# daooshee/ReReVST-Code

Hardware: AMD Instinct MI355X
Metric: stylized frames/sec at 512x512, 1 style (higher is better)
Workload: dtype f32

## Files before the change

### rerevst-code_amd/csrc/rerevst_hip.hip

```cpp
#include <hip/hip_runtime.h>
#include <dlfcn.h>
#include <stddef.h>
#include <stdint.h>
#include <string.h>
#include <algorithm>
#include <cmath>
#include <thread>
#include <stdio.h>
#include <map>
#include <condition_variable>
#include <mutex>
#include <string>
#include <vector>

#include "../../include/rerevst_hip.h"
#include "conv_mfma.h"
#include "conv_wino.h"
#include "conv_wino_split.h"
#include "conv_f43.h"
#include "conv_thin.h"
#include "prep_kernels.h"
#include "mask_kernels.h"

namespace {
// ... 174 lines not shown
    struct Ticket { long id = -1; void* out = nullptr; size_t out_bytes = 0; bool open = false; } tickets[4];
    long next_ticket = 0;
    int grid_share = 1;
    int f43_mode = 1;
    unsigned f43_layers = F43_DEFAULT_LAYERS;
    bool illcond = false;
    bool enc_p8_tables = false;
    int p8 = 3;
    bool f43_path = false;
    unsigned direct_layers = 0;
    int ms_group = 0;
    int host_io = 0;
    int n_cus = 256;
    int debug = 0;
    int fail_alloc_in = 0;
    bool profiling = false;
    std::vector<ProfEntry> prof;
};

namespace {

#define HIPCHK(expr)                                                                              \
    do {                                                                                          \
        hipError_t _e = (expr);                                                                   \
        if (_e != hipSuccess) {                                                                   \
            char _b[512];                                                                         \
            snprintf(_b, sizeof _b, "%s failed: %s (%s:%d)", #expr, hipGetErrorString(_e), __FILE__, __LINE__); \
            h->err = _b;                                                                          \
            return _e == hipErrorOutOfMemory ? RRV_E_NOMEM : RRV_E_HIP;                           \
        }                                                                                         \
    } while (0)
#define RCHK(expr) do { int _r = (expr); if (_r != RRV_OK) return _r; } while (0)

int fail(rrv_handle h, int code, const std::string& msg) { h->err = msg; return code; }
int dmalloc(rrv_handle h, void** p, size_t bytes);

int check_image_size(rrv_handle h, double H, double W, const char* who) {
    if ((H + 2) * (W + 2) * 64.0 < 2147483648.0) return RRV_OK;
    return fail(h, RRV_E_ARG, std::string(who) + ": frame too large ((H+2)*(W+2)*64 must be < 2^31)");
}
int check_frame(rrv_handle h, int H, int W, const char* who) {
    if (H < 8 || W < 8) return fail(h, RRV_E_ARG, std::string(who) + ": frames must be at least 8 x 8 pixels");
    return check_image_size(h, H, W, who);
}

int sync_all(rrv_handle h) {
    for (int i = 0; i < RRV_MAX_SLOTS; ++i)
        if (h->streams[i]) HIPCHK(hipStreamSynchronize(h->streams[i]));
    if (h->copy_in) HIPCHK(hipStreamSynchronize(h->copy_in));
    if (h->copy_out) HIPCHK(hipStreamSynchronize(h->copy_out));
    return RRV_OK;
}

int dmalloc(rrv_handle h, void** p, size_t bytes) {
    *p = nullptr;
    if (h->fail_alloc_in > 0 && --h->fail_alloc_in == 0) {
        char b[160];
        snprintf(b, sizeof b, "out of device memory (injected by rrv_debug_fail_alloc) allocating %zu bytes", bytes);
        return fail(h, RRV_E_NOMEM, b);
    }
    const hipError_t e = hipMalloc(p, bytes);
    if (e != hipSuccess) {
        (void)hipGetLastError();
        *p = nullptr;
        char b[200];
        snprintf(b, sizeof b, "hipMalloc of %zu bytes failed: %s", bytes, hipGetErrorString(e));
        return fail(h, e == hipErrorOutOfMemory ? RRV_E_NOMEM : RRV_E_HIP, b);
    }
    return RRV_OK;
}

int dalloc(rrv_handle h, float** p, size_t floats, bool zero = true) {
    RCHK(dmalloc(h, (void**)p, floats * sizeof(float)));
    if (zero) HIPCHK(hipMemsetAsync(*p, 0, floats * sizeof(float), h->stream));
    return RRV_OK;
}

constexpr size_t DBG_GUARD = 16384;
constexpr uint32_t DBG_CANARY = 0xDEADBEEFu;
struct DbgRec { rrv_ctx* h; float* base; int B, H, W, C; size_t floats; };
std::mutex g_dbg_mu;
std::map<float*, DbgRec> g_dbg;

__global__ void dbg_check_k(const float* base, const float* p, int B, int H, int W, int C, size_t floats, unsigned* counters) {
    const uint32_t* gb = (const uint32_t*)base;
    const uint32_t* u = (const uint32_t*)p;
    const size_t img = (size_t)(H + 2) * (W + 2) * C;
    const size_t tid = blockIdx.x * (size_t)blockDim.x + threadIdx.x, nth = (size_t)gridDim.x * blockDim.x;
    unsigned bad_guard = 0, bad_ring = 0;
    for (size_t i = tid; i < DBG_GUARD; i += nth) bad_guard += (gb[i] != DBG_CANARY) + (((const uint32_t*)(p + floats))[i] != DBG_CANARY);
    const size_t ring_px = (size_t)2 * (W + 2) + (size_t)2 * H;
    for (size_t i = tid; i < (size_t)B * ring_px * C; i += nth) {
        const size_t c = i % C, r = (i / C) % ring_px, b = i / C / ring_px;
        size_t y, x;
        if (r < (size_t)(W + 2)) { y = 0; x = r; }
        else if (r < (size_t)2 * (W + 2)) { y = H + 1; x = r - (W + 2); }
        else { const size_t q = r - 2 * (W + 2); y = 1 + (q >> 1); x = (q & 1) ? W + 1 : 0; }
        bad_ring += u[b * img + (y * (W + 2) + x) * C + c] != 0u;
    }
    for (size_t i = (size_t)B * img + tid; i < floats; i += nth) bad_ring += u[i] != 0u;
    if (bad_guard) atomicAdd(&counters[0], bad_guard);
    if (bad_ring) atomicAdd(&counters[1], bad_ring);
}
__global__ void dbg_fill_k(uint32_t* p, size_t n, uint32_t v) {
    for (size_t i = blockIdx.x * (size_t)blockDim.x + threadIdx.x; i < n; i += (size_t)gridDim.x * blockDim.x) p[i] = v;
}
// ... 1217 lines not shown
    if (rc == RRV_OK && h->debug) rc = debug_verify(h, "Decoder.compute (streaming)");
    (void)hipStreamSynchronize(h->stream);
    h->active_src = -1;
    if (rc == RRV_OK) S.computed = true;
    if (rc == RRV_OK) rc = filter_conditioning(h, S);
    return rc;
}

}

extern "C" {

static int cu_mask_count(const char* env, int device, int n_cus) {
    if (!env || !*env) return 0;
    auto parse_list = [](const char* b, const char* e, int limit, std::vector<char>& hit) {
        hit.assign((size_t)limit, 0);
        while (b < e) {
            char* q = nullptr;
            long lo = strtol(b, &q, 10), hi = lo;
            if (q == b) return false;
            if (q < e && *q == '-') { const char* r = q + 1; hi = strtol(r, &q, 10); if (q == r) return false; }
            for (long v = lo; v <= hi; ++v) if (v >= 0 && v < limit) hit[(size_t)v] = 1;
            b = (q < e && *q == ',') ? q + 1 : q;
            if (b < e && q == b) return false;
        }
        return true;
    };
    const char* p = env;
    while (*p) {
        const char* semi = strchr(p, ';');
        const char* end = semi ? semi : p + strlen(p);
        const char* colon = (const char*)memchr(p, ':', (size_t)(end - p));
        if (colon) {
            std::vector<char> gpus, cus;
            if (parse_list(p, colon, 64, gpus) && device < 64 && gpus[(size_t)device] && parse_list(colon + 1, end, n_cus, cus)) {
                int n = 0;
                for (char c : cus) n += c;
                return n;
            }
        }
        p = semi ? semi + 1 : end;
    }
    return 0;
}

int rrv_create(int device, rrv_handle* out) {
    if (!out) return RRV_E_ARG;
    *out = nullptr;
    int n = 0;
    if (hipGetDeviceCount(&n) != hipSuccess || device < 0 || device >= n) return RRV_E_HIP;
    rrv_ctx* h = new rrv_ctx();
    h->dev = device;
    bool ok = hipSetDevice(device) == hipSuccess;
    for (int i = 0; ok && i < RRV_MAX_SLOTS; ++i) ok = hipStreamCreateWithFlags(&h->streams[i], hipStreamNonBlocking) == hipSuccess;
    if (!ok) {
        delete h;
        return RRV_E_HIP;
    }
    h->stream = h->streams[0];
    ok = ok && hipStreamCreateWithFlags(&h->copy_in, hipStreamNonBlocking) == hipSuccess && hipStreamCreateWithFlags(&h->copy_out, hipStreamNonBlocking) == hipSuccess;
    for (int i = 0; ok && i < RRV_MAX_SLOTS; ++i) ok = hipEventCreateWithFlags(&h->slot_ev[i], hipEventDisableTiming) == hipSuccess;
    for (auto& st : h->hstage)
        for (hipEvent_t* e : {&st.in_done, &st.k_done, &st.out_done}) ok = ok && hipEventCreateWithFlags(e, hipEventDisableTiming) == hipSuccess;
    for (const ConvKey& e : WINO_TABLE)
        if (ok && e.attr) ok = e.attr() == hipSuccess;
    for (const ConvKey& e : F43_TABLE)
        if (ok && e.attr) ok = e.attr() == hipSuccess;
    for (const F43LayKey& e : F43_LAY_TABLE)
        if (ok && e.attr) ok = e.attr() == hipSuccess;
    if (!ok) {
        delete h;
        return RRV_E_HIP;
    }
    {
        hipDeviceProp_t prop;
        if (hipGetDeviceProperties(&prop, device) == hipSuccess && prop.multiProcessorCount > 0) h->n_cus = prop.multiProcessorCount;
        const int masked = cu_mask_count(getenv("HSA_CU_MASK"), device, h->n_cus);
        if (masked > 0 && masked < h->n_cus) h->n_cus = masked;
        if (const char* e = getenv("RRV_CUS")) { const int n = atoi(e); if (n >= 1 && n <= 1024) h->n_cus = n; }
    }
    if (const char* e = getenv("RRV_F43_LAYERS")) h->f43_layers = (unsigned)strtoul(e, nullptr, 0);
    if (const char* e = getenv("RRV_DIRECT_LAYERS")) h->direct_layers = (unsigned)strtoul(e, nullptr, 0);
    if (const char* e = getenv("RRV_P8")) h->p8 = atoi(e) & 3;
    if (const char* e = getenv("RRV_F43")) h->f43_mode = atoi(e) < 0 ? 0 : (atoi(e) > 2 ? 2 : atoi(e));
    if (const char* e = getenv("RRV_DEBUG")) h->debug = atoi(e) < 0 ? 0 : (atoi(e) > 2 ? 2 : atoi(e));
    *out = h;
    return RRV_OK;
}

static void free_plans(rrv_handle h) {
    for (auto& pair : h->enc_frame) for (EncPlan& e : pair) enc_free(e);
    enc_free(h->enc_add); enc_free(h->enc_style);
    for (auto& pair : h->dec) for (DecPlan& d : pair) dec_free(h, d);
    prep_free(h);
}

int rrv_set_debug(rrv_handle h, int level) {
    if (!h || level < 0 || level > 2) return RRV_E_ARG;
    HIPCHK(hipSetDevice(h->dev));
    RCHK(sync_all(h));
    free_plans(h);
    h->debug = level;
    return RRV_OK;
}

int rrv_debug_fail_alloc(rrv_handle h, int nth) {
    if (!h || nth < 0) return RRV_E_ARG;
    h->fail_alloc_in = nth;
    return RRV_OK;
}

__global__ void dbg_poke_k(float* p, long off) { p[off] = 1.0f; }
int rrv_debug_selftest(rrv_handle h) {
    if (!h) return RRV_E_ARG;
// ... 16 lines not shown
    h->debug = saved;
    if (rc != RRV_OK) return rc;
    if (caught != 2) return fail(h, RRV_E_DEBUG, "debug selftest: a deliberate out-of-bounds store was not detected");
    h->err.clear();
    return RRV_OK;
}

int rrv_destroy(rrv_handle h) {
    if (!h) return RRV_E_ARG;
    (void)hipSetDevice(h->dev);
    (void)hipDeviceSynchronize();
    for (auto& kv : h->conv) {
        if (kv.second.raw) (void)hipFree(kv.second.raw);
        if (kv.second.pk) (void)hipFree(kv.second.pk);
        if (kv.second.pk_ups) (void)hipFree(kv.second.pk_ups);
        if (kv.second.pk_ups_sc) (void)hipFree(kv.second.pk_ups_sc);
        if (kv.second.pk_wino) (void)hipFree(kv.second.pk_wino);
        if (kv.second.pk_f43) (void)hipFree(kv.second.pk_f43);
        if (kv.second.bias && kv.second.bias != h->zero_bias) (void)hipFree(kv.second.bias);
    }
    if (h->zero_bias) (void)hipFree(h->zero_bias);
    for (int f = 0; f < 3; ++f) {
        const ConvW &fd = h->sets[0].fold_down[f], &fu = h->sets[0].fold_up[f];
        for (float* q : {fd.raw, fd.bias, fd.pk_wino, fu.raw, fu.pk_wino}) if (q) (void)hipFree(q);
    }
    if (h->sets[0].active) (void)hipFree(h->sets[0].active);
    for (int i = 0; i < 6; ++i) { if (h->fc_w[i]) (void)hipFree(h->fc_w[i]); if (h->fc_b[i]) (void)hipFree(h->fc_b[i]); }
    if (h->fold_tmp) (void)hipFree(h->fold_tmp);
    for (float* p : h->patches) (void)hipFree(p);
    for (auto& f : h->features) if (f.owned) { if (f.p) (void)hipFree(f.p); if (f.u8) (void)hipFree(f.u8); }
    for (void* b : h->feat_blocks) (void)hipFree(b);
    free_plans(h);
    for (StyleState& s : h->styles) { if (s.blob) (void)hipFree(s.blob); if (s.smean) (void)hipFree(s.smean); tfree(&s.map); }
    if (h->d_u8) (void)hipFree(h->d_u8);
    if (h->d_outf) (void)hipFree(h->d_outf);
    if (h->pend_u8) (void)hipFree(h->pend_u8);
    for (auto& bw : h->blend_w) {
        if (bw.dev) (void)hipFree(bw.dev);
        if (bw.pin) (void)hipHostFree(bw.pin);
        for (hipEvent_t e : bw.ev) if (e) (void)hipEventDestroy(e);
    }
    if (h->stat_part) (void)hipFree(h->stat_part);
    for (float* q : {h->first_w[0], h->first_w[1], h->first_b[0], h->first_b[1], h->first_wg}) if (q) (void)hipFree(q);
    for (auto& st : h->hstage) {
        stage_free(st.pin, true);
        stage_free(st.dev, false);
        if (st.mask) (void)hipFree(st.mask);
        if (st.mask_pin) (void)hipHostFree(st.mask_pin);
        for (hipEvent_t e : {st.in_done, st.k_done, st.out_done}) if (e) (void)hipEventDestroy(e);
    }
    if (h->copy_in) (void)hipStreamDestroy(h->copy_in);
    if (h->copy_out) (void)hipStreamDestroy(h->copy_out);
    for (ProfEntry& e : h->prof) { (void)hipEventDestroy(e.e0); (void)hipEventDestroy(e.e1); }
    for (int i = 0; i < RRV_MAX_SLOTS; ++i) { (void)hipStreamDestroy(h->streams[i]); if (h->slot_ev[i]) (void)hipEventDestroy(h->slot_ev[i]); }
    delete h;
    return RRV_OK;
}

const char* rrv_last_error(rrv_handle h) { return h ? h->err.c_str() : "null handle"; }

int rrv_load_weight(rrv_handle h, const char* key, const float* data, const int64_t* shape, int ndim) {
    if (!h || !key || !data || !shape || ndim < 1 || ndim > 4) return RRV_E_ARG;
    if (h->finalized) return fail(h, RRV_E_WEIGHTS, "weights already finalized");
    size_t n = 1;
    for (int i = 0; i < ndim; ++i) n *= (size_t)shape[i];
    h->hostw[key].assign(data, data + n);
    h->hostshape[key].assign(shape, shape + ndim);
    return RRV_OK;
}

int rrv_finalize_weights(rrv_handle h) {
    if (!h) return RRV_E_ARG;
    if (h->finalized) return RRV_OK;
    HIPCHK(hipSetDevice(h->dev));
    RCHK(dalloc(h, &h->zero_bias, 512, true));
    {
        constexpr size_t PART = (size_t)1024 * 3 * 512, ACC = (size_t)2 * 4 * 512, FLOATS = 512 + 64;
        float* base;
        RCHK(dalloc(h, &base, (2 * PART + ACC) * 2 + FLOATS));
        h->stat_part = (double*)base; h->stat_part2 = h->stat_part + PART; h->stat_acc = h->stat_part2 + PART;
        h->stat_mean = (float*)(h->stat_acc + ACC); h->prep_cmean = h->stat_mean + 512;
    }
    for (int which = 0; which < 2; ++which) {
        for (int i = 0; i < 9; ++i) {
            char k[64];
            if (which == 0) snprintf(k, sizeof k, "Encoder.slice.%d", VGG_IDX[i]);
            else snprintf(k, sizeof k, "EncoderStyle.slice%d.%d", STYLE_SLICE[i], VGG_IDX[i]);
            if (i == 0) {
                float* raw = nullptr;
                RCHK(upload(h, std::string(k) + ".weight", &raw, 64 * 27));
                RCHK(dalloc(h, &h->first_w[which], 27 * 64, false));
                hipLaunchKernelGGL(pack_first_k, dim3(7), dim3(256), 0, h->stream, (const float*)raw, h->first_w[which]);
                HIPCHK(hipGetLastError());
                RCHK(upload(h, std::string(k) + ".bias", &h->first_b[which], 64));
                if (which == 0) {
                    RCHK(dalloc(h, &h->first_wg, 1216, false));
                    hipLaunchKernelGGL(pack_first_grey_k, dim3(3), dim3(256), 0, h->stream, (const float*)raw, (const float*)h->first_b[0], h->first_wg);
                    HIPCHK(hipGetLastError());
                }
                HIPCHK(hipStreamSynchronize(h->stream));
                (void)hipFree(raw);
            } else {
                RCHK(make_conv(h, k, VGG_COUT[i], VGG_CIN[i], 9, true));
                if (which == 0 && i < 8) { h->conv[k].f43_bit = i - 1; RCHK(pack_f43(h, h->conv[k])); }
            }
        }
    }
// ... 685 lines not shown
    pool->run((char*)dst, (const char*)src, bytes, nt, slice);
}
static std::mutex g_pin_mu;
static std::map<const char*, size_t> g_pin_ranges;
static bool is_pinned(const void* ptr, size_t bytes) {
    {
        std::lock_guard<std::mutex> lk(g_pin_mu);
        auto it = g_pin_ranges.upper_bound((const char*)ptr);
        if (it != g_pin_ranges.begin()) {
            --it;
            if ((const char*)ptr + bytes <= it->first + it->second) return true;
        }
    }
    hipPointerAttribute_t a;
    for (const char* q : {(const char*)ptr, (const char*)ptr + (bytes ? bytes - 1 : 0)}) {
        if (hipPointerGetAttributes(&a, q) != hipSuccess) { (void)hipGetLastError(); return false; }
        if (a.type != hipMemoryTypeHost) return false;
    }
    return true;
}
static int retire_ticket(rrv_handle h, int set);
static int claim_staging(rrv_handle h) {
    for (int i = 0; i < HOST_SETS; ++i) RCHK(retire_ticket(h, i));
    RCHK(sync_all(h));
    h->next_slot = 0;
    return RRV_OK;
}
static int host_pipeline(rrv_handle h, const uint8_t* frames, void* out, const Xfer& x) {
    if (!h || !frames || !out) return RRV_E_ARG;
    HIPCHK(hipSetDevice(h->dev));
    RCHK(check_xfer(h, x, true));
    const int B = x.B;
    const float* const mask = x.mask;
    const int mask_images = x.mask_images;
    const size_t fb = x.in_bytes(h);
    const size_t fob = x.out_elems() * out_elem(x.fmt);
    char* const outc = (char*)out;
    const int sub = x.model == Model::GLOBAL ? host_sub(B, x.KH(), x.KW()) : std::min(host_sub(B, x.KH(), x.KW()), (int)rrv_ctx::MS_GROUP_MAX);
    const size_t mfl = x.mask_floats();
    auto run = [&](int slot, int k, const void* d_in, int nb, void* d_out) -> int {
        Xfer part = x;
        part.B = nb;
        if (x.wts) part.wts = x.wts + (size_t)k * sub * x.ns;
        if (mask) { part.mask = h->hstage[k % HOST_SETS].mask; part.mask_images = mask_images == 1 ? 1 : nb; }
        return run_xfer(h, slot, d_in, d_out, part);
    };
    const bool in_pin = is_pinned(frames, (size_t)B * fb), out_pin = is_pinned(out, (size_t)B * fob);
    const size_t msub = (size_t)(mask_images == 1 ? 1 : sub) * mfl;
    const bool m_pin = mask && is_pinned(mask, (size_t)mask_images * mfl * sizeof(float));
    const bool host_in = !in_pin || (mask && !m_pin);
    RCHK(claim_staging(h));
    const int nchunk = (B + sub - 1) / sub;
    const int nsets = nchunk < HOST_SETS ? nchunk : HOST_SETS;
    const bool zin = h->host_io == 1 || h->host_io == 2, zout = h->host_io == 1 || h->host_io == 3;
    for (int i = 0; i < nsets; ++i) {
        RCHK(stage_reserve(h, i, zin ? 0 : (size_t)sub * fb, zout ? 0 : (size_t)sub * fob, false));
        RCHK(stage_reserve(h, i, in_pin ? 0 : (size_t)sub * fb, out_pin ? 0 : (size_t)sub * fob, true));
        if (!mask) continue;
        rrv_ctx::HostStage& st = h->hstage[i];
        RCHK(ensure_dev(h, st.mask, st.mask_cap, msub));
        if (!m_pin && st.mask_pin_cap < msub) {
            if (st.mask_pin) (void)hipHostFree(st.mask_pin);
            st.mask_pin = nullptr; st.mask_pin_cap = 0;
            if (hipHostMalloc((void**)&st.mask_pin, msub * sizeof(float), hipHostMallocDefault) != hipSuccess) {
                (void)hipGetLastError();
                st.mask_pin = nullptr;
                return fail(h, RRV_E_NOMEM, "staging: out of page-locked host memory");
            }
            st.mask_pin_cap = msub;
        }
    }
    auto count = [&](int k) { return (k + 1) * sub <= B ? sub : B - k * sub; };
    auto drain = [&](int k) -> int {
        auto& st = h->hstage[k % HOST_SETS];
        HIPCHK(hipEventSynchronize(st.out_done));
        if (!out_pin) host_copy(outc + (size_t)k * sub * fob, st.pin.out, (size_t)count(k) * fob);
        return RRV_OK;
    };
    int rc = RRV_OK;
    for (int k = 0; k < nchunk && rc == RRV_OK; ++k) {
        auto& st = h->hstage[k % HOST_SETS];
        const bool reuse = k >= HOST_SETS;
        if (reuse && (host_in || !out_pin)) rc = drain(k - HOST_SETS);
        if (rc != RRV_OK) break;
        const int nb = count(k);
        const uint8_t* src = frames + (size_t)k * sub * fb;
        if (!in_pin) { host_copy(st.pin.in, src, (size_t)nb * fb); src = st.pin.in; }
        const float* msrc = nullptr;
        size_t mbytes = 0;
        if (mask) {
            msrc = mask + (mask_images == 1 ? 0 : (size_t)k * sub * mfl);
            mbytes = (size_t)(mask_images == 1 ? 1 : nb) * mfl * sizeof(float);
            if (!m_pin) { host_copy(st.mask_pin, msrc, mbytes); msrc = st.mask_pin; }
        }
        const int slot = h->profiling ? 0 : (k & 1) % h->n_slots;
        hipStream_t cs = h->streams[slot];
        if (nchunk == 1 && h->host_io == 0) {
            HIPCHK(hipMemcpyAsync(st.dev.in, src, (size_t)nb * fb, hipMemcpyHostToDevice, cs));
            if (mask) HIPCHK(hipMemcpyAsync(st.mask, msrc, mbytes, hipMemcpyHostToDevice, cs));
            rc = run(slot, k, st.dev.in, nb, st.dev.out);
            if (rc != RRV_OK) break;
            HIPCHK(hipMemcpyAsync(out_pin ? out : st.pin.out, st.dev.out, (size_t)nb * fob, hipMemcpyDeviceToHost, cs));
            HIPCHK(hipStreamSynchronize(cs));
            if (!out_pin) host_copy(out, st.pin.out, (size_t)nb * fob);
            return RRV_OK;
        }
        const uint8_t* k_in = src;
        if (!zin || mask) {
            if (reuse) HIPCHK(hipStreamWaitEvent(h->copy_in, st.k_done, 0));
            if (!zin) {
                HIPCHK(hipMemcpyAsync(st.dev.in, src, (size_t)nb * fb, hipMemcpyHostToDevice, h->copy_in));
                k_in = st.dev.in;
            }
            if (mask) HIPCHK(hipMemcpyAsync(st.mask, msrc, mbytes, hipMemcpyHostToDevice, h->copy_in));
            HIPCHK(hipEventRecord(st.in_done, h->copy_in));
            HIPCHK(hipStreamWaitEvent(cs, st.in_done, 0));
        }
        void* const h_dst = out_pin ? outc + (size_t)k * sub * fob : st.pin.out;
        if (reuse) HIPCHK(hipStreamWaitEvent(cs, st.out_done, 0));
        void* const k_out = zout ? h_dst : st.dev.out;
        rc = run(slot, k, k_in, nb, k_out);
        if (rc != RRV_OK) break;
        if (!zin || mask) HIPCHK(hipEventRecord(st.k_done, cs));
        if (zout) { HIPCHK(hipEventRecord(st.out_done, cs)); continue; }
        if (zin && !mask) HIPCHK(hipEventRecord(st.k_done, cs));
        HIPCHK(hipStreamWaitEvent(h->copy_out, st.k_done, 0));
        HIPCHK(hipMemcpyAsync(h_dst, st.dev.out, (size_t)nb * fob, hipMemcpyDeviceToHost, h->copy_out));
        HIPCHK(hipEventRecord(st.out_done, h->copy_out));
    }
    if (rc != RRV_OK) { (void)sync_all(h); return rc; }
    const int first_open = (host_in || !out_pin) ? (nchunk - HOST_SETS < 0 ? 0 : nchunk - HOST_SETS) : 0;
    if (!host_in && out_pin) {
        if (zout) RCHK(sync_all(h));
        else HIPCHK(hipStreamSynchronize(h->copy_out));
    } else {
        for (int k = first_open; k < nchunk; ++k) RCHK(drain(k));
    }
    return RRV_OK;
}

int rrv_transfer(rrv_handle h, const uint8_t* frame, int H, int W, float* out) {
    return host_pipeline(h, frame, out, Xfer{Model::GLOBAL, 1, H, W, PLAIN, OUT_F32});
}
int rrv_transfer_u8(rrv_handle h, const uint8_t* frame, int H, int W, uint8_t* out) {
    return host_pipeline(h, frame, out, Xfer{Model::GLOBAL, 1, H, W, PLAIN, OUT_U8});
}

int rrv_transfer_batch(rrv_handle h, const uint8_t* frames, int B, int H, int W, float* out) {
    return host_pipeline(h, frames, out, Xfer{Model::GLOBAL, B, H, W, PLAIN, OUT_F32});
}
int rrv_transfer_batch_u8(rrv_handle h, const uint8_t* frames, int B, int H, int W, uint8_t* out) {
    return host_pipeline(h, frames, out, Xfer{Model::GLOBAL, B, H, W, PLAIN, OUT_U8});
}

int rrv_transfer_frames(rrv_handle h, const uint8_t* frames, int B, int H, int W, float* out) {
    return host_pipeline(h, frames, out, Xfer{Model::GLOBAL, B, H, W, PADDED, OUT_F32});
}
int rrv_transfer_frames_u8(rrv_handle h, const uint8_t* frames, int B, int H, int W, uint8_t* out) {
    return host_pipeline(h, frames, out, Xfer{Model::GLOBAL, B, H, W, PADDED, OUT_U8});
}

int rrv_transfer_blend_batch(rrv_handle h, const uint8_t* frames, int B, int H, int W, const float* wts, int ns, int pad_crop, float* out) {
    return host_pipeline(h, frames, out, Xfer{Model::BLEND, B, H, W, pad_crop != 0, OUT_F32, ns, wts});
}
int rrv_transfer_blend_batch_u8(rrv_handle h, const uint8_t* frames, int B, int H, int W, const float* wts, int ns, int pad_crop, uint8_t* out) {
    return host_pipeline(h, frames, out, Xfer{Model::BLEND, B, H, W, pad_crop != 0, OUT_U8, ns, wts});
}

int rrv_transfer_mask_batch(rrv_handle h, const uint8_t* frames, int B, int H, int W, const float* mask, int ns, int mask_images, int pad_crop, float* out) {
    return host_pipeline(h, frames, out, Xfer{Model::MASK, B, H, W, pad_crop != 0, OUT_F32, ns,  nullptr, mask, mask_images});
}
int rrv_transfer_mask_batch_u8(rrv_handle h, const uint8_t* frames, int B, int H, int W, const float* mask, int ns, int mask_images, int pad_crop, uint8_t* out) {
    return host_pipeline(h, frames, out, Xfer{Model::MASK, B, H, W, pad_crop != 0, OUT_U8, ns,  nullptr, mask, mask_images});
}

int rrv_transfer_frame_mode_batch(rrv_handle h, const uint8_t* frames, int B, int H, int W, float* out) {
    return host_pipeline(h, frames, out, Xfer{Model::FRAME, B, H, W, PLAIN, OUT_F32});
}
int rrv_transfer_frame_mode_batch_u8(rrv_handle h, const uint8_t* frames, int B, int H, int W, uint8_t* out) {
    return host_pipeline(h, frames, out, Xfer{Model::FRAME, B, H, W, PLAIN, OUT_U8});
}

int rrv_transfer_frame_mode_frames(rrv_handle h, const uint8_t* frames, int B, int H, int W, float* out) {
    return host_pipeline(h, frames, out, Xfer{Model::FRAME, B, H, W, PADDED, OUT_F32});
}
int rrv_transfer_frame_mode_frames_u8(rrv_handle h, const uint8_t* frames, int B, int H, int W, uint8_t* out) {
    return host_pipeline(h, frames, out, Xfer{Model::FRAME, B, H, W, PADDED, OUT_U8});
}

static int retire_ticket(rrv_handle h, int set) {
    auto& tk = h->tickets[set];
    if (!tk.open) return RRV_OK;
    HIPCHK(hipEventSynchronize(h->hstage[set].out_done));
    if (tk.out) host_copy(tk.out, h->hstage[set].pin.out, tk.out_bytes);
    tk.open = false;
    return RRV_OK;
}

static int transfer_async(rrv_handle h, const uint8_t* frame, int H, int W, void* out, OutFmt fmt, long* ticket) {
    if (!h || !frame || !out || !ticket) return RRV_E_ARG;
    RCHK(check_frame(h, H, W, "transfer"));
    HIPCHK(hipSetDevice(h->dev));
    const size_t fb = (size_t)H * W * 3, fo = (size_t)(H / 8 * 8) * (W / 8 * 8) * 3 * out_elem(fmt);
    const long id = h->next_ticket;
    const int set = (int)(id % HOST_SETS);
    auto& st = h->hstage[set];
    RCHK(retire_ticket(h, set));
    const bool in_pin = is_pinned(frame, fb), out_pin = is_pinned(out, fo);
    RCHK(stage_reserve(h, set, in_pin ? 0 : fb, out_pin ? 0 : fo, true));
    RCHK(stage_reserve(h, set, fb, 0, false));
    const uint8_t* src = frame;
    if (!in_pin) { host_copy(st.pin.in, frame, fb); src = st.pin.in; }
    const int slot = h->profiling ? 0 : (int)(id % RRV_MAX_SLOTS);
    h->next_slot = 0;
    hipStream_t cs = h->streams[slot];
    struct ShareScope { rrv_handle h; int saved; ~ShareScope() { h->grid_share = saved; } } share_scope{h, h->grid_share};
    if (!h->profiling && h->grid_share == 1) {
        int open = 1;
        for (auto& tk : h->tickets)
            if (tk.open && tk.id != id - HOST_SETS && hipEventQuery(h->hstage[tk.id % HOST_SETS].out_done) == hipErrorNotReady) ++open;
        (void)hipGetLastError();
        h->grid_share = open > RRV_MAX_SLOTS ? RRV_MAX_SLOTS : open;
    }
    RCHK(ensure_active(h));
    HIPCHK(hipMemcpyAsync(st.dev.in, src, fb, hipMemcpyHostToDevice, cs));
    HIPCHK(hipEventRecord(st.in_done, cs));
    const int rc0 = transfer_device(h, slot, st.dev.in, 1, H, W, out_pin ? out : st.pin.out, fmt);
    if (in_pin) HIPCHK(hipEventSynchronize(st.in_done));
    if (rc0 != RRV_OK) return rc0;
    HIPCHK(hipEventRecord(st.out_done, cs));
    auto& tk0 = h->tickets[set];
    tk0.id = id; tk0.out = out_pin ? nullptr : out; tk0.out_bytes = fo; tk0.open = true;
    h->next_ticket = id + 1;
    *ticket = id;
    return RRV_OK;
}
int rrv_transfer_async(rrv_handle h, const uint8_t* frame, int H, int W, float* out, long* ticket) {
    return transfer_async(h, frame, H, W, out, OUT_F32, ticket);
}
int rrv_transfer_async_u8(rrv_handle h, const uint8_t* frame, int H, int W, uint8_t* out, long* ticket) {
    return transfer_async(h, frame, H, W, out, OUT_U8, ticket);
}

int rrv_transfer_wait(rrv_handle h, long ticket) {
    if (!h) return RRV_E_ARG;
    if (ticket < 0 || ticket >= h->next_ticket) return fail(h, RRV_E_ARG, "transfer_wait: no such ticket");
    HIPCHK(hipSetDevice(h->dev));
    const int set = (int)(ticket % HOST_SETS);
    if (h->tickets[set].id != ticket) {
        if (h->tickets[set].id > ticket) return RRV_OK;
        return fail(h, RRV_E_ARG, "transfer_wait: unknown ticket");
    }
    return retire_ticket(h, set);
}

static size_t feature_floats(int H, int W) {
    const int fh = H / 8, fw = W / 8;
    return (size_t)(fh + 2) * (fw + 2) * 512 + (size_t)20 * (fw + 2 + 20) * 512;
}

int rrv_generate_content_features(rrv_handle h, const uint8_t* frame, int H, int W, int* feature_id) {
    if (!h || !frame || !feature_id) return RRV_E_ARG;
    if (!h->finalized) return fail(h, RRV_E_WEIGHTS, "weights not finalized");
    RCHK(check_frame(h, H, W, "generate_content_features"));
    HIPCHK(hipSetDevice(h->dev));
    RCHK(sync_all(h));
    rrv_ctx::Feature ft{nullptr, H, W, nullptr, true};
    const size_t need = feature_floats(H, W) * sizeof(float);
    if (h->feat_bytes + need > h->feat_cap) {
        RCHK(dmalloc(h, (void**)&ft.u8, (size_t)H * W * 3));
        HIPCHK(hipMemcpy(ft.u8, frame, (size_t)H * W * 3, hipMemcpyHostToDevice));
        h->features.push_back(ft);
        *feature_id = (int)h->features.size() - 1;
        return RRV_OK;
    }
    RCHK(ensure_dev(h, h->d_u8, h->d_u8_cap, (size_t)H * W * 3));
    HIPCHK(hipMemcpyAsync(h->d_u8, frame, (size_t)H * W * 3, hipMemcpyHostToDevice, h->stream));
    RCHK(enc_plan(h, h->enc_add, 1, H, W));
    RCHK(run_encoder(h, h->enc_add, h->d_u8, 0, nullptr, nullptr, 1));
    const Tens& f = h->enc_add.c41;
    RCHK(dalloc(h, &ft.p, feature_floats(H, W), true));
    HIPCHK(hipMemcpyAsync(ft.p, f.p, f.img_floats() * sizeof(float), hipMemcpyDeviceToDevice, h->stream));
    HIPCHK(hipStreamSynchronize(h->stream));
    h->feat_bytes += need;
    h->features.push_back(ft);
    *feature_id = (int)h->features.size() - 1;
    return RRV_OK;
}

int rrv_generate_content_features_batch(rrv_handle h, const uint8_t* frames, int B, int H, int W, int* feature_ids) {
    if (!h || !frames || !feature_ids || B < 1) return RRV_E_ARG;
    if (!h->finalized) return fail(h, RRV_E_WEIGHTS, "weights not finalized");
    RCHK(check_frame(h, H, W, "generate_content_features"));
    HIPCHK(hipSetDevice(h->dev));
    RCHK(claim_staging(h));
    const size_t fb = (size_t)H * W * 3;
    Tens one; one.B = 1; one.H = H / 8; one.W = W / 8; one.C = 512;
    const size_t img = one.img_floats(), slack = feature_floats(H, W) - img;
    int n_res = 0;
    while (n_res < B && h->feat_bytes + ((size_t)(n_res + 1) * img + slack) * sizeof(float) <= h->feat_cap) ++n_res;
    const int id0 = (int)h->features.size();
    const size_t bytes0 = h->feat_bytes, blocks0 = h->feat_blocks.size();
    float* arena = nullptr;
    auto work = [&]() -> int {
    if (n_res) {
        RCHK(dmalloc(h, (void**)&arena, ((size_t)n_res * img + slack) * sizeof(float)));
        h->feat_blocks.push_back(arena);
        HIPCHK(hipMemsetAsync(arena, 0, ((size_t)n_res * img + slack) * sizeof(float), h->streams[0]));
        HIPCHK(hipStreamSynchronize(h->streams[0]));
        h->feat_bytes += ((size_t)n_res * img + slack) * sizeof(float);
        for (int i = 0; i < n_res; ++i) h->features.push_back(rrv_ctx::Feature{arena + (size_t)i * img, H, W, nullptr, false});
    }
    if (n_res < B) {
        uint8_t* blk = nullptr;
        RCHK(dmalloc(h, (void**)&blk, (size_t)(B - n_res) * fb));
        h->feat_blocks.push_back(blk);
        HIPCHK(hipMemcpy(blk, frames + (size_t)n_res * fb, (size_t)(B - n_res) * fb, hipMemcpyHostToDevice));
        for (int i = n_res; i < B; ++i) h->features.push_back(rrv_ctx::Feature{nullptr, H, W, blk + (size_t)(i - n_res) * fb, false});
    }
    for (int i = 0; i < B; ++i) feature_ids[i] = id0 + i;
    if (!n_res) return RRV_OK;
    const int sub = host_sub(n_res, H, W);
    const int nchunk = (n_res + sub - 1) / sub;
    const int nsets = nchunk < HOST_SETS ? nchunk : HOST_SETS;
    const bool in_pin = is_pinned(frames, (size_t)n_res * fb);
    for (int i = 0; i < nsets; ++i) {
        RCHK(stage_reserve(h, i, (size_t)sub * fb, 0, false));
        RCHK(stage_reserve(h, i, in_pin ? 0 : (size_t)sub * fb, 0, true));
    }
    struct Restore { rrv_handle h; ~Restore() { h->stream = h->streams[0]; h->f43_path = false; } } restore{h};
    const int nstreams = (h->profiling || h->n_slots < 2) ? 1 : 2;
    int rc = RRV_OK;
    for (int k = 0; k < nchunk && rc == RRV_OK; ++k) {
        auto& st = h->hstage[k % HOST_SETS];
        const int nb = (k + 1) * sub <= n_res ? sub : n_res - k * sub;
        const uint8_t* src = frames + (size_t)k * sub * fb;
        if (k >= HOST_SETS) HIPCHK(hipEventSynchronize(st.k_done));
        if (!in_pin) { host_copy(st.pin.in, src, (size_t)nb * fb); src = st.pin.in; }
        const int slot = k % nstreams;
        HIPCHK(hipMemcpyAsync(st.dev.in, src, (size_t)nb * fb, hipMemcpyHostToDevice, h->copy_in));
        HIPCHK(hipEventRecord(st.in_done, h->copy_in));
        HIPCHK(hipStreamWaitEvent(h->streams[slot], st.in_done, 0));
        h->stream = h->streams[slot];
        h->f43_path = true;
        EncPlan& e = pick_plan(h, h->enc_frame[slot], nb, H, W);
        rc = enc_plan(h, e, nb, H, W, true);
        if (rc != RRV_OK) break;
        e.gen = ++h->launch_gen;
// ... 44 lines not shown
    const rrv_ctx::Feature& ft = h->features[feature_id];
    if (!h->patches.empty() && (ft.H != h->add_H || ft.W != h->add_W))
        return fail(h, RRV_E_ARG, "add_patch: all sampled features must have the same size");
    Tens f; f.B = 1; f.H = ft.H / 2 / 2 / 2; f.W = ft.W / 2 / 2 / 2; f.C = 512;
    float* keep = nullptr;
    RCHK(dalloc(h, &keep, f.img_floats(), false));
    const float* src = ft.p;
    if (!src) {
        int rc = enc_plan(h, h->enc_add, 1, ft.H, ft.W);
        if (rc == RRV_OK) rc = run_encoder(h, h->enc_add, ft.u8, 0, nullptr, nullptr, 1);
        if (rc == RRV_OK && hipStreamSynchronize(h->stream) != hipSuccess) rc = fail(h, RRV_E_HIP, "add_patch: encoder failed");
        if (rc != RRV_OK) { (void)hipFree(keep); return rc; }
        src = h->enc_add.c41.p;
    }
    HIPCHK(hipMemcpy(keep, src, f.img_floats() * sizeof(float), hipMemcpyDeviceToDevice));
    h->patches.push_back(keep);
    h->patch_h = f.H; h->patch_w = f.W; h->add_H = ft.H; h->add_W = ft.W;
    return RRV_OK;
}

static int transfer_features(rrv_handle h, int feature_id, const float* wts, int ns, void* out, OutFmt fmt) {
    if (!h || !wts || !out || ns < 1 || ns > RRV_MAX_STYLES) return RRV_E_ARG;
    if (feature_id < 0 || feature_id >= (int)h->features.size() || !(h->features[feature_id].p || h->features[feature_id].u8)) return RRV_E_ARG;
    HIPCHK(hipSetDevice(h->dev));
    RCHK(sync_all(h));
    h->next_slot = 0;
    const rrv_ctx::Feature& ft = h->features[feature_id];
    RCHK(blend_into_current(h, wts, ns));
    const size_t n = (size_t)(ft.H / 8 * 8) * (ft.W / 8 * 8) * 3;
    RCHK(ensure_dev(h, h->d_outf, h->d_outf_cap, out_floats(n, fmt)));
    RCHK(transfer_device(h, 0, ft.u8, 1, ft.H, ft.W, h->d_outf, fmt, ft.p));
    HIPCHK(hipMemcpyAsync(out, h->d_outf, n * out_elem(fmt), hipMemcpyDeviceToHost, h->streams[0]));
    HIPCHK(hipStreamSynchronize(h->streams[0]));
    return RRV_OK;
}
int rrv_transfer_features(rrv_handle h, int feature_id, const float* wts, int ns, float* out) {
    return transfer_features(h, feature_id, wts, ns, out, OUT_F32);
}
int rrv_transfer_features_u8(rrv_handle h, int feature_id, const float* wts, int ns, uint8_t* out) {
    return transfer_features(h, feature_id, wts, ns, out, OUT_U8);
}

static int transfer_features_batch(rrv_handle h, const int* ids, const float* wts, int n, int ns, void* out, OutFmt fmt) {
    if (!h || !ids || !wts || !out || n < 1 || ns < 1 || ns > RRV_MAX_STYLES) return RRV_E_ARG;
    HIPCHK(hipSetDevice(h->dev));
    for (int i = 0; i < n; ++i)
        if (ids[i] < 0 || ids[i] >= (int)h->features.size() || !(h->features[ids[i]].p || h->features[ids[i]].u8)) return fail(h, RRV_E_ARG, "transfer: unknown feature id");
    for (int s = 0; s < ns; ++s)
        if (!h->styles[s].computed) return fail(h, RRV_E_STATE, "blend: state not computed for every style");
    const int H = h->features[ids[0]].H, W = h->features[ids[0]].W;
    for (int i = 1; i < n; ++i)
        if (h->features[ids[i]].H != H || h->features[ids[i]].W != W) return fail(h, RRV_E_ARG, "transfer: features of one call must share their size");
    RCHK(claim_staging(h));
    const size_t npx = (size_t)(H / 8 * 8) * (W / 8 * 8) * 3 * out_elem(fmt);
    char* const outc = (char*)out;
    const bool out_pin = is_pinned(out, (size_t)n * npx);
    int G = h->ms_group;
    if (G == 0) {
        const long s = HOST_SUB_PIXELS / ((long)H * W);
        G = s < 1 ? 1 : s > rrv_ctx::MS_GROUP_MAX ? rrv_ctx::MS_GROUP_MAX : (int)s;
    }
    if (G > n) G = n;
    struct Group { int first, count; };
    std::vector<Group> groups;
    for (int i = 0; i < n;) {
        if (!h->features[ids[i]].p) { groups.push_back({i, 1}); ++i; continue; }
        int c = 0;
        while (c < G && i + c < n && h->features[ids[i + c]].p) ++c;
        groups.push_back({i, c});
        i += c;
    }
    const int ngroups = (int)groups.size();
    const int nslots = (h->profiling || h->n_slots < 2 || ngroups < 2) ? 1 : 2;
    for (int i = 0; i < nslots; ++i) {
        RCHK(stage_reserve(h, i, 0, (size_t)G * npx, false));
        RCHK(stage_reserve(h, i, 0, out_pin ? 0 : (size_t)G * npx, true));
    }
    SetScope scope{h, -2};
    auto drain = [&](int k) -> int {
        auto& st = h->hstage[k % nslots];
        HIPCHK(hipEventSynchronize(st.out_done));
        if (!out_pin) host_copy(outc + (size_t)groups[k].first * npx, st.pin.out, (size_t)groups[k].count * npx);
        return RRV_OK;
    };
    for (int k = 0; k < ngroups; ++k) {
        const int slot = k % nslots, first = groups[k].first, cnt = groups[k].count;
        auto& st = h->hstage[slot];
        if (k >= nslots) {
            if (!out_pin) RCHK(drain(k - nslots));
            HIPCHK(hipStreamWaitEvent(h->streams[slot], st.out_done, 0));
        }
        h->stream = h->streams[slot];
        const float* fp[rrv_ctx::MS_GROUP_MAX] = {};
        h->cur = &h->sets[rrv_ctx::MS_GROUP_MAX * slot];
        {
            static_assert(rrv_ctx::MS_GROUP_MAX <= 16, "BlendManyP::w holds sixteen images");
            BlendManyP bp{};
            bp.n = ns; bp.out = h->cur->active; bp.count = RRV_STATE_FLOATS;
            for (int s = 0; s < ns; ++s) bp.st[s] = h->styles[s].blob;
            for (int g = 0; g < cnt; ++g) {
                for (int s = 0; s < ns; ++s) bp.w[g][s] = wts[(size_t)(first + g) * ns + s];
                fp[g] = h->features[ids[first + g]].p;
            }
            hipLaunchKernelGGL(blend_states_k, dim3((RRV_STATE_FLOATS + 255) / 256, cnt), dim3(256), 0, h->stream, bp);
            HIPCHK(hipGetLastError());
            for (int f = 0; f < 3; ++f) RCHK(fold_filters(h, h->cur->active, f, cnt));
// ... 35 lines not shown
    h->feat_blocks.clear();
    h->features.clear();
    h->feat_bytes = 0;
    return RRV_OK;
}

static int transfer_frame_mode(rrv_handle h, const uint8_t* frame, int H, int W, void* out, OutFmt fmt) {
    if (!h || !frame || !out) return RRV_E_ARG;
    if (!h->finalized) return fail(h, RRV_E_WEIGHTS, "weights not finalized");
    RCHK(check_frame(h, H, W, "transfer"));
    HIPCHK(hipSetDevice(h->dev));
    StyleState& S = h->styles[0];
    if (!S.prepared) return fail(h, RRV_E_STATE, "prepare_style has not been called");
    RCHK(sync_all(h));
    const size_t nin = (size_t)H * W * 3;
    const size_t n = (size_t)(H / 8 * 8) * (W / 8 * 8) * 3;
    RCHK(ensure_dev(h, h->d_u8, h->d_u8_cap, nin));
    HIPCHK(hipMemcpyAsync(h->d_u8, frame, nin, hipMemcpyHostToDevice, h->stream));
    RCHK(ensure_dev(h, h->d_outf, h->d_outf_cap, out_floats(n, fmt)));
    RCHK(frame_mode_device(h, 0, h->d_u8, 1, H, W, h->d_outf, fmt, nullptr));
    HIPCHK(hipMemcpyAsync(out, h->d_outf, n * out_elem(fmt), hipMemcpyDeviceToHost, h->streams[0]));
    HIPCHK(hipStreamSynchronize(h->streams[0]));
    return RRV_OK;
}
int rrv_transfer_frame_mode(rrv_handle h, const uint8_t* frame, int H, int W, float* out) {
    return transfer_frame_mode(h, frame, H, W, out, OUT_F32);
}
int rrv_transfer_frame_mode_u8(rrv_handle h, const uint8_t* frame, int H, int W, uint8_t* out) {
    return transfer_frame_mode(h, frame, H, W, out, OUT_U8);
}

int rrv_get_preclamp_image(rrv_handle h, float* out, int H, int W, int b) {
    if (!h || !out) return RRV_E_ARG;
    if (!h->last_pre || h->last_pre_H != H || h->last_pre_W != W) return fail(h, RRV_E_STATE, "get_preclamp: no transfer of that size yet");
    if (b < 0 || b >= h->last_pre_B) return fail(h, RRV_E_ARG, "get_preclamp: the last launch had fewer images");
    HIPCHK(hipSetDevice(h->dev));
    RCHK(sync_all(h));
    HIPCHK(hipMemcpy(out, h->last_pre + (size_t)b * H * W * 3, (size_t)H * W * 3 * sizeof(float), hipMemcpyDeviceToHost));
    return RRV_OK;
}

int rrv_get_preclamp(rrv_handle h, float* out, int H, int W) { return rrv_get_preclamp_image(h, out, H, W, 0); }

int rrv_sync(rrv_handle h) {
    if (!h) return RRV_E_ARG;
    HIPCHK(hipSetDevice(h->dev));
    return sync_all(h);
}

int rrv_set_pipeline(rrv_handle h, int n_slots) {
    if (!h || n_slots < 1 || n_slots > RRV_MAX_SLOTS) return RRV_E_ARG;
    HIPCHK(hipSetDevice(h->dev));
    RCHK(sync_all(h));
    h->n_slots = n_slots;
    h->next_slot = 0;
    return RRV_OK;
}

int rrv_set_grid_share(rrv_handle h, int share) {
    if (!h || share < 1 || share > 4) return RRV_E_ARG;
    h->grid_share = share;
    return RRV_OK;
}

int rrv_set_f43(rrv_handle h, int mode) {
    if (!h || mode < 0 || mode > 2) return RRV_E_ARG;
    RCHK(sync_all(h));
    h->f43_mode = mode;
    return RRV_OK;
}

int rrv_set_multistyle_group(rrv_handle h, int frames) {
    if (!h || frames < 0 || frames > rrv_ctx::MS_GROUP_MAX) return RRV_E_ARG;
    h->ms_group = frames;
    return RRV_OK;
}

int rrv_set_host_io(rrv_handle h, int mode) {
    if (!h || mode < 0 || mode > 3) return RRV_E_ARG;
    HIPCHK(hipSetDevice(h->dev));
    for (int i = 0; i < 4; ++i) RCHK(retire_ticket(h, i));
    RCHK(sync_all(h));
    h->host_io = mode;
    return RRV_OK;
}

static int tap_row(int index, bool& enc) {
    enc = index < 9 || (index >= 23 && index < 30);
    return index < 9 ? index : index < 23 ? index - 9 : index < 30 ? index - 14 : index - 16;
}

int rrv_debug_copy_tensor(rrv_handle h, int slot, int index, int H, int W, float* host, size_t cap, size_t* floats) {
    if (!h || slot < 0 || slot >= RRV_MAX_SLOTS || index < 0 || index > 22 || !floats) return RRV_E_ARG;
    HIPCHK(hipSetDevice(h->dev));
    RCHK(sync_all(h));
    bool enc;
    const int row = tap_row(index, enc);
    const Tens* t = nullptr;
    for (int k = 0; k < 2 && !t; ++k) {
        EncPlan& e = h->enc_frame[slot][k]; DecPlan& d = h->dec[slot][k];
        if (enc ? (e.H == H && e.W == W && e.B > 0) : (d.H == H / 8 * 8 && d.W == W / 8 * 8 && d.B > 0)) t = enc ? &ENC_T[row].of(e) : &DEC_T[row].of(d);
    }
    if (!t || !t->p) return fail(h, RRV_E_STATE, "debug_copy_tensor: no such tensor in this slot");
    *floats = t->img_floats();
    if (host && cap >= *floats) HIPCHK(hipMemcpy(host, t->p, *floats * sizeof(float), hipMemcpyDeviceToHost));
    return RRV_OK;
// ... 126 lines not shown
```

Before: 839.7.

## Lazily create streams and defer D2H copies two chunks behind kernel launches

Slot streams, slot events and the copy streams are now created on demand instead of all at handle creation, which trims setup work and leaves fewer idle queues. In the chunked host transfer path, the device-to-host copy of each chunk is issued two iterations later, after a host wait on that chunk's kernel-done event. The aim is to keep the copy queue from stalling on cross-stream waits and to let kernels run ahead of the copies. The price is host-side blocking on event sync, plus extra bookkeeping to ensure streams exist on every entry point.

```diff
diff --git a/rerevst-code_amd/csrc/rerevst_hip.hip b/rerevst-code_amd/csrc/rerevst_hip.hip
--- a/rerevst-code_amd/csrc/rerevst_hip.hip
+++ b/rerevst-code_amd/csrc/rerevst_hip.hip
@@ -250,6 +250,38 @@
     return RRV_OK;
 }
 
+int ensure_slot_streams(rrv_handle h, int n) {
+    hipStream_t s[RRV_MAX_SLOTS] = {nullptr};
+    hipEvent_t e[RRV_MAX_SLOTS] = {nullptr};
+    hipError_t err = hipSuccess;
+    for (int i = 0; i < n && err == hipSuccess; ++i) {
+        if (!h->streams[i]) err = hipStreamCreateWithFlags(&s[i], hipStreamNonBlocking);
+        if (err == hipSuccess && !h->slot_ev[i]) err = hipEventCreateWithFlags(&e[i], hipEventDisableTiming);
+    }
+    if (err != hipSuccess) {
+        (void)hipGetLastError();
+        for (int i = 0; i < n; ++i) { if (s[i]) (void)hipStreamDestroy(s[i]); if (e[i]) (void)hipEventDestroy(e[i]); }
+        return fail(h, err == hipErrorOutOfMemory ? RRV_E_NOMEM : RRV_E_HIP, std::string("stream creation failed: ") + hipGetErrorString(err));
+    }
+    for (int i = 0; i < n; ++i) { if (s[i]) h->streams[i] = s[i]; if (e[i]) h->slot_ev[i] = e[i]; }
+    return RRV_OK;
+}
+int ensure_copy_streams(rrv_handle h) {
+    if (h->copy_in && h->copy_out) return RRV_OK;
+    hipStream_t in = nullptr, out = nullptr;
+    hipError_t err = h->copy_in ? hipSuccess : hipStreamCreateWithFlags(&in, hipStreamNonBlocking);
+    if (err == hipSuccess && !h->copy_out) err = hipStreamCreateWithFlags(&out, hipStreamNonBlocking);
+    if (err != hipSuccess) {
+        (void)hipGetLastError();
+        if (in) (void)hipStreamDestroy(in);
+        if (out) (void)hipStreamDestroy(out);
+        return fail(h, err == hipErrorOutOfMemory ? RRV_E_NOMEM : RRV_E_HIP, std::string("stream creation failed: ") + hipGetErrorString(err));
+    }
+    if (in) h->copy_in = in;
+    if (out) h->copy_out = out;
+    return RRV_OK;
+}
+
 int dmalloc(rrv_handle h, void** p, size_t bytes) {
     *p = nullptr;
     if (h->fail_alloc_in > 0 && --h->fail_alloc_in == 0) {
@@ -1573,14 +1605,12 @@
     rrv_ctx* h = new rrv_ctx();
     h->dev = device;
     bool ok = hipSetDevice(device) == hipSuccess;
-    for (int i = 0; ok && i < RRV_MAX_SLOTS; ++i) ok = hipStreamCreateWithFlags(&h->streams[i], hipStreamNonBlocking) == hipSuccess;
+    ok = ok && ensure_slot_streams(h, 2) == RRV_OK;
     if (!ok) {
         delete h;
         return RRV_E_HIP;
     }
     h->stream = h->streams[0];
-    ok = ok && hipStreamCreateWithFlags(&h->copy_in, hipStreamNonBlocking) == hipSuccess && hipStreamCreateWithFlags(&h->copy_out, hipStreamNonBlocking) == hipSuccess;
-    for (int i = 0; ok && i < RRV_MAX_SLOTS; ++i) ok = hipEventCreateWithFlags(&h->slot_ev[i], hipEventDisableTiming) == hipSuccess;
     for (auto& st : h->hstage)
         for (hipEvent_t* e : {&st.in_done, &st.k_done, &st.out_done}) ok = ok && hipEventCreateWithFlags(e, hipEventDisableTiming) == hipSuccess;
     for (const ConvKey& e : WINO_TABLE)
@@ -1703,7 +1733,7 @@
     if (h->copy_in) (void)hipStreamDestroy(h->copy_in);
     if (h->copy_out) (void)hipStreamDestroy(h->copy_out);
     for (ProfEntry& e : h->prof) { (void)hipEventDestroy(e.e0); (void)hipEventDestroy(e.e1); }
-    for (int i = 0; i < RRV_MAX_SLOTS; ++i) { (void)hipStreamDestroy(h->streams[i]); if (h->slot_ev[i]) (void)hipEventDestroy(h->slot_ev[i]); }
+    for (int i = 0; i < RRV_MAX_SLOTS; ++i) { if (h->streams[i]) (void)hipStreamDestroy(h->streams[i]); if (h->slot_ev[i]) (void)hipEventDestroy(h->slot_ev[i]); }
     delete h;
     return RRV_OK;
 }
@@ -2495,6 +2525,7 @@
     RCHK(claim_staging(h));
     const int nchunk = (B + sub - 1) / sub;
     const int nsets = nchunk < HOST_SETS ? nchunk : HOST_SETS;
+    if (nchunk > 1 || h->host_io != 0) RCHK(ensure_copy_streams(h));
     const bool zin = h->host_io == 1 || h->host_io == 2, zout = h->host_io == 1 || h->host_io == 3;
     for (int i = 0; i < nsets; ++i) {
         RCHK(stage_reserve(h, i, zin ? 0 : (size_t)sub * fb, zout ? 0 : (size_t)sub * fob, false));
@@ -2518,6 +2549,15 @@
         auto& st = h->hstage[k % HOST_SETS];
         HIPCHK(hipEventSynchronize(st.out_done));
         if (!out_pin) host_copy(outc + (size_t)k * sub * fob, st.pin.out, (size_t)count(k) * fob);
+        return RRV_OK;
+    };
+    constexpr int PACE_AHEAD = 2;
+    static_assert(PACE_AHEAD < HOST_SETS, "a set's D2H copy is queued before the set is drained and reused");
+    auto deliver = [&](int j) -> int {
+        auto& sj = h->hstage[j % HOST_SETS];
+        HIPCHK(hipEventSynchronize(sj.k_done));
+        HIPCHK(hipMemcpyAsync(out_pin ? (void*)(outc + (size_t)j * sub * fob) : sj.pin.out, sj.dev.out, (size_t)count(j) * fob, hipMemcpyDeviceToHost, h->copy_out));
+        HIPCHK(hipEventRecord(sj.out_done, h->copy_out));
         return RRV_OK;
     };
     int rc = RRV_OK;
@@ -2550,7 +2590,7 @@
         }
         const uint8_t* k_in = src;
         if (!zin || mask) {
-            if (reuse) HIPCHK(hipStreamWaitEvent(h->copy_in, st.k_done, 0));
+            if (reuse && zout) HIPCHK(hipStreamWaitEvent(h->copy_in, st.k_done, 0));
             if (!zin) {
                 HIPCHK(hipMemcpyAsync(st.dev.in, src, (size_t)nb * fb, hipMemcpyHostToDevice, h->copy_in));
                 k_in = st.dev.in;
@@ -2564,13 +2604,11 @@
         void* const k_out = zout ? h_dst : st.dev.out;
         rc = run(slot, k, k_in, nb, k_out);
         if (rc != RRV_OK) break;
-        if (!zin || mask) HIPCHK(hipEventRecord(st.k_done, cs));
+        if (!zin || mask || !zout) HIPCHK(hipEventRecord(st.k_done, cs));
         if (zout) { HIPCHK(hipEventRecord(st.out_done, cs)); continue; }
-        if (zin && !mask) HIPCHK(hipEventRecord(st.k_done, cs));
-        HIPCHK(hipStreamWaitEvent(h->copy_out, st.k_done, 0));
-        HIPCHK(hipMemcpyAsync(h_dst, st.dev.out, (size_t)nb * fob, hipMemcpyDeviceToHost, h->copy_out));
-        HIPCHK(hipEventRecord(st.out_done, h->copy_out));
-    }
+        if (k >= PACE_AHEAD) rc = deliver(k - PACE_AHEAD);
+    }
+    for (int j = nchunk < PACE_AHEAD ? 0 : nchunk - PACE_AHEAD; !zout && j < nchunk && rc == RRV_OK; ++j) rc = deliver(j);
     if (rc != RRV_OK) { (void)sync_all(h); return rc; }
     const int first_open = (host_in || !out_pin) ? (nchunk - HOST_SETS < 0 ? 0 : nchunk - HOST_SETS) : 0;
     if (!host_in && out_pin) {
@@ -2655,6 +2693,7 @@
     const uint8_t* src = frame;
     if (!in_pin) { host_copy(st.pin.in, frame, fb); src = st.pin.in; }
     const int slot = h->profiling ? 0 : (int)(id % RRV_MAX_SLOTS);
+    RCHK(ensure_slot_streams(h, slot + 1));
     h->next_slot = 0;
     hipStream_t cs = h->streams[slot];
     struct ShareScope { rrv_handle h; int saved; ~ShareScope() { h->grid_share = saved; } } share_scope{h, h->grid_share};
@@ -2737,6 +2776,7 @@
     RCHK(check_frame(h, H, W, "generate_content_features"));
     HIPCHK(hipSetDevice(h->dev));
     RCHK(claim_staging(h));
+    RCHK(ensure_copy_streams(h));
     const size_t fb = (size_t)H * W * 3;
     Tens one; one.B = 1; one.H = H / 8; one.W = W / 8; one.C = 512;
     const size_t img = one.img_floats(), slack = feature_floats(H, W) - img;
@@ -2887,6 +2927,7 @@
     for (int i = 1; i < n; ++i)
         if (h->features[ids[i]].H != H || h->features[ids[i]].W != W) return fail(h, RRV_E_ARG, "transfer: features of one call must share their size");
     RCHK(claim_staging(h));
+    RCHK(ensure_copy_streams(h));
     const size_t npx = (size_t)(H / 8 * 8) * (W / 8 * 8) * 3 * out_elem(fmt);
     char* const outc = (char*)out;
     const bool out_pin = is_pinned(out, (size_t)n * npx);
@@ -3028,6 +3069,7 @@
     if (!h || n_slots < 1 || n_slots > RRV_MAX_SLOTS) return RRV_E_ARG;
     HIPCHK(hipSetDevice(h->dev));
     RCHK(sync_all(h));
+    RCHK(ensure_slot_streams(h, n_slots));
     h->n_slots = n_slots;
     h->next_slot = 0;
     return RRV_OK;
```

New measurement: 846.8, median of 6. Within noise of the previous version (+0.8%).
